# nico-franco-gomez/dsptoolbox

Measured on AMD Instinct MI355X. Metric: Msamples/s + GB/s vs HBM roofline, 64ch Welch H1 nfft=4096 @1/2/4/8 GPU, higher is better.
Workload: dtype f32

## Files before the change

### dsptoolbox_amd/csrc/kernels_welch4096.hpp

```cpp
#pragma once
#include <hip/hip_runtime.h>
#include <stdint.h>

#include <cmath>
#include <utility>
#include <vector>

#include "kernels_finish.hpp"

namespace welch4096 {

#ifndef W4_ABLATE
#define W4_ABLATE 0
#endif

#ifndef W4_AB
#define W4_AB 0
#endif

#ifndef W4_TIMING
#define W4_TIMING 0
#endif
#if W4_TIMING
__device__ unsigned long long w4_timing[16];
#define W4_TS(i)                                                  \
    do {                                                          \
        __builtin_amdgcn_sched_barrier(0);                        \
        unsigned long long t_ = __builtin_amdgcn_s_memtime();     \
        __builtin_amdgcn_sched_barrier(0);                        \
        if ((i) > 0) w4_ph[(i)-1] += t_ - w4_prev;                \
        w4_prev = t_;                                             \
    } while (0)
#else
#define W4_TS(i)
#endif

constexpr int N = 4096, NT = 256, NB = N / 2 + 1;
constexpr int L1S = 272, L2S = 18;
constexpr int BUF_C = 256 * L2S;
constexpr int LDS_BYTES = BUF_C * 8 + 256 * 8;
constexpr int LDS_BYTES_2 = 2 * BUF_C * 8 + 256 * 8;

__device__ __forceinline__ float2 cmul(float2 a, float2 b) {
    return make_float2(fmaf(a.x, b.x, -a.y * b.y), fmaf(a.x, b.y, a.y * b.x));
}

__device__ __forceinline__ void r4(float2& a, float2& b, float2& c, float2& d) {
    float2 s0 = make_float2(a.x + c.x, a.y + c.y), d0 = make_float2(a.x - c.x, a.y - c.y);
    float2 s1 = make_float2(b.x + d.x, b.y + d.y), d1 = make_float2(b.x - d.x, b.y - d.y);
    a = make_float2(s0.x + s1.x, s0.y + s1.y);
    c = make_float2(s0.x - s1.x, s0.y - s1.y);
    b = make_float2(d0.x + d1.y, d0.y - d1.x);
    d = make_float2(d0.x - d1.y, d0.y + d1.x);
}

__device__ __forceinline__ void dft16(float2 (&v)[16]) {
    constexpr float C8 = 0.92387953251128673848f, S8 = 0.38268343236508978178f;
    constexpr float R2 = 0.70710678118654752440f;
#pragma unroll
    for (int n0 = 0; n0 < 4; ++n0) r4(v[n0], v[n0 + 4], v[n0 + 8], v[n0 + 12]);
    auto mulw = [](float2 z, float c, float s) {
        return make_float2(fmaf(z.x, c, z.y * s), fmaf(z.y, c, -z.x * s));
    };
    v[1 + 4] = mulw(v[1 + 4], C8, S8);
    v[1 + 8] = make_float2((v[9].x + v[9].y) * R2, (v[9].y - v[9].x) * R2);
    v[1 + 12] = mulw(v[1 + 12], S8, C8);
    v[2 + 4] = make_float2((v[6].x + v[6].y) * R2, (v[6].y - v[6].x) * R2);
    v[2 + 8] = make_float2(v[10].y, -v[10].x);
    v[2 + 12] = make_float2((v[14].y - v[14].x) * R2, -(v[14].x + v[14].y) * R2);
    v[3 + 4] = mulw(v[3 + 4], S8, C8);
    v[3 + 8] = make_float2((v[11].y - v[11].x) * R2, -(v[11].x + v[11].y) * R2);
    v[3 + 12] = mulw(v[3 + 12], -C8, -S8);
#pragma unroll
    for (int k1 = 0; k1 < 4; ++k1) r4(v[4 * k1], v[4 * k1 + 1], v[4 * k1 + 2], v[4 * k1 + 3]);
}
__device__ __forceinline__ constexpr int pos16(int k) { return 4 * (k & 3) + (k >> 2); }

#define W4_PIN() __builtin_amdgcn_sched_barrier(0)
template <typename PA, typename HA, typename HB>
__device__ __forceinline__ void dft16_h(float2 (&v)[16], PA pre_a, HA after_a, HB after_b) {
    constexpr float C8 = 0.92387953251128673848f, S8 = 0.38268343236508978178f;
    constexpr float R2 = 0.70710678118654752440f;
    auto mulw = [](float2 z, float c, float s) {
        return make_float2(fmaf(z.x, c, z.y * s), fmaf(z.y, c, -z.x * s));
    };
    pre_a(std::integral_constant<int, 0>{});
    r4(v[0], v[4], v[8], v[12]);
    after_a(0);
    pre_a(std::integral_constant<int, 1>{});
    r4(v[1], v[5], v[9], v[13]);
    if (!(W4_AB & 16)) {
    v[5] = mulw(v[5], C8, S8);
    v[9] = make_float2((v[9].x + v[9].y) * R2, (v[9].y - v[9].x) * R2);
    v[13] = mulw(v[13], S8, C8);
    }
    after_a(1);
    pre_a(std::integral_constant<int, 2>{});
    r4(v[2], v[6], v[10], v[14]);
    if (!(W4_AB & 16)) {
    v[6] = make_float2((v[6].x + v[6].y) * R2, (v[6].y - v[6].x) * R2);
    v[10] = make_float2(v[10].y, -v[10].x);
    v[14] = make_float2((v[14].y - v[14].x) * R2, -(v[14].x + v[14].y) * R2);
    }
    after_a(2);
    pre_a(std::integral_constant<int, 3>{});
    r4(v[3], v[7], v[11], v[15]);
    if (!(W4_AB & 16)) {
    v[7] = mulw(v[7], S8, C8);
    v[11] = make_float2((v[11].y - v[11].x) * R2, -(v[11].x + v[11].y) * R2);
    v[15] = mulw(v[15], -C8, -S8);
    }
    after_a(3);
#pragma unroll
    for (int g = 0; g < 4; ++g) {
        r4(v[4 * g], v[4 * g + 1], v[4 * g + 2], v[4 * g + 3]);
        after_b(g);
    }
}
struct NoHookI {
    template <typename T>
    __device__ __forceinline__ void operator()(T) const {}
};


struct Tw {
    float2 w[15];
};

struct NoHook {
    __device__ __forceinline__ void operator()() const {}
};
template <bool TWO_BUF, typename Hook = NoHook, typename Hook2 = NoHook>
__device__ __forceinline__ void fft4096(float2 (&v)[16], const Tw& tw, float2* __restrict__ buf,
                                        const float2* __restrict__ tw2, int tid
#if W4_TIMING
                                        , unsigned long long (&w4_ph)[12], unsigned long long& w4_prev
#endif
                                        , Hook behind_ex1 = Hook(), Hook2 behind_ex2 = Hook2()) {
    float2* __restrict__ bufB = TWO_BUF ? buf + BUF_C : buf;
    dft16(v);
#pragma unroll
    for (int k1 = 1; k1 < 16; ++k1) v[pos16(k1)] = cmul(v[pos16(k1)], tw.w[k1 - 1]);
    W4_TS(2);
    const int k1u = tid >> 4, n3 = tid & 15;
    if (!(W4_ABLATE & 4)) {
        if (!TWO_BUF) __syncthreads();
#pragma unroll
        for (int k1 = 0; k1 < 16; ++k1) buf[k1 * L1S + tid] = v[pos16(k1)];
    }
    float2 w2[15];
#pragma unroll
    for (int k2 = 1; k2 < 16; ++k2) w2[k2 - 1] = tw2[k2 * 16 + n3];
    behind_ex1();
    if (!(W4_ABLATE & 4)) {
        W4_TS(3);
        __syncthreads();
        W4_TS(4);
#pragma unroll
        for (int n2 = 0; n2 < 16; ++n2) v[n2] = buf[k1u * L1S + 16 * n2 + n3];
    }
    W4_TS(5);
    dft16(v);
#pragma unroll
    for (int k2 = 1; k2 < 16; ++k2) v[pos16(k2)] = cmul(v[pos16(k2)], w2[k2 - 1]);
    W4_TS(6);
    if (!(W4_ABLATE & 4)) {
        if (!TWO_BUF) __syncthreads();
#pragma unroll
        for (int k2 = 0; k2 < 16; ++k2) bufB[(16 * k2 + k1u) * L2S + n3] = v[pos16(k2)];
        behind_ex2();
        W4_TS(7);
        __syncthreads();
        W4_TS(8);
        const float4* row = reinterpret_cast<const float4*>(bufB + tid * L2S);
#pragma unroll
        for (int j = 0; j < 8; ++j) {
            float4 r = row[j];
            v[2 * j] = make_float2(r.x, r.y);
            v[2 * j + 1] = make_float2(r.z, r.w);
        }
    }
    W4_TS(9);
    dft16(v);
    W4_TS(10);
}

template <bool TWO_BUF>
__device__ __forceinline__ void fft4096_plain(float2 (&v)[16], const Tw& tw, float2* __restrict__ buf,
                                              const float2* __restrict__ tw2, int tid) {
#if W4_TIMING
    unsigned long long ph[12] = {}, prev = 0;
    fft4096<TWO_BUF>(v, tw, buf, tw2, tid, ph, prev);
#else
    fft4096<TWO_BUF>(v, tw, buf, tw2, tid);
#endif
}

struct Args {
    const float* sig;
    int64_t n_samples, ld;
    int n_ch, hop, n_frames, n_pairs, detrend;
    int n_chunks, ppc;
    const float* window;
    const float2* twt;
    float2* xs;
    float* px;
    float2* pxy;
    float* pyy;
    float* psx;
    int use_plus;
    uint32_t plus[24];
    int n_cx;
    const float* xsig;
};

constexpr int TWT_LEN = 15 * 256 + 256;
__device__ __forceinline__ void init_tables(Tw& tw, float (&win)[16], float2* tw2,
                                            const float* __restrict__ window,
                                            const float2* __restrict__ twt, int tid) {
#pragma unroll
    for (int k1 = 1; k1 < 16; ++k1) tw.w[k1 - 1] = twt[(k1 - 1) * 256 + tid];
#pragma unroll
    for (int n1 = 0; n1 < 16; ++n1) win[n1] = window[tid + 256 * n1];
    tw2[tid] = twt[15 * 256 + tid];
    __syncthreads();
}
inline void host_tables(std::vector<float2>& t) {
    t.resize(TWT_LEN);
    for (int k1 = 1; k1 < 16; ++k1)
        for (int tt = 0; tt < 256; ++tt) {
            double a = -2.0 * M_PI * (double)(tt * k1) / 4096.0;
            t[(k1 - 1) * 256 + tt] = make_float2((float)std::cos(a), (float)std::sin(a));
        }
    for (int k2 = 0; k2 < 16; ++k2)
        for (int n3 = 0; n3 < 16; ++n3) {
            double a = -2.0 * M_PI * (double)(n3 * k2) / 256.0;
            t[15 * 256 + k2 * 16 + n3] = make_float2((float)std::cos(a), (float)std::sin(a));
        }
}

template <bool HALF_HOP>
struct Raw {
    float s[HALF_HOP ? 24 : 32];
};

template <bool HALF_HOP>
__device__ __forceinline__ void load_raw(Raw<HALF_HOP>& r, const float* __restrict__ ch,
                                         int64_t n_samples, int64_t start0, int hop, int tid) {
    const float* __restrict__ src = ch + start0;
    const int64_t remain = n_samples - start0;
    const int span = HALF_HOP ? 3 * 2048 : hop + 4096;
    if (remain >= span) {
        if (HALF_HOP) {
#pragma unroll
            for (int m = 0; m < 24; ++m) r.s[m] = src[tid + 256 * m];
        } else {
#pragma unroll
            for (int n1 = 0; n1 < 16; ++n1) {
                r.s[n1] = src[tid + 256 * n1];
                r.s[16 + n1] = src[hop + tid + 256 * n1];
            }
        }
    } else {
        const int last = (int)(remain > (int64_t)(1 << 30) ? (1 << 30) : remain) - 1;
        constexpr int CNT = HALF_HOP ? 24 : 32;
#pragma unroll
        for (int m = 0; m < CNT; ++m) {
            int i = HALF_HOP ? tid + 256 * m : (m < 16 ? tid + 256 * m : hop + tid + 256 * (m - 16));
            float a = src[min(i, last)];
            r.s[m] = i <= last ? a : 0.f;
        }
    }
}

template <bool HALF_HOP>
__device__ __forceinline__ void window_pair(float2 (&v)[16], const Raw<HALF_HOP>& r, const float (&win)[16]) {
#pragma unroll
    for (int n1 = 0; n1 < 16; ++n1) {
        float b = HALF_HOP ? r.s[n1 + 8] : r.s[16 + n1];
        v[n1] = make_float2(r.s[n1] * win[n1], b * win[n1]);
    }
}

__device__ __forceinline__ bool needs_drop(const Args& p, int pr) {
    return pr == p.n_pairs - 1 && (p.n_frames & 1) && (int64_t)p.n_frames * p.hop < p.n_samples;
}
__device__ __forceinline__ void drop_second(float2 (&v)[16]) {
#pragma unroll
    for (int n1 = 0; n1 < 16; ++n1) v[n1].y = 0.f;
}

template <bool HALF_HOP>
__global__ __launch_bounds__(NT) void k_x(Args p) {
    extern __shared__ __align__(16) float2 lds[];
    float2* buf = lds;
    float2* tw2 = lds + BUF_C;
    const int tid = threadIdx.x, pr = blockIdx.x, cx = blockIdx.y;
    Tw tw;
    float win[16];
    float2 v[16];
    {
        Raw<HALF_HOP> raw;
        load_raw<HALF_HOP>(raw, p.sig + (int64_t)cx * p.ld, p.n_samples, (int64_t)(2 * pr) * p.hop, p.hop, tid);
        init_tables(tw, win, tw2, p.window, p.twt, tid);
        window_pair<HALF_HOP>(v, raw, win);
        if (needs_drop(p, pr)) drop_second(v);
    }
    fft4096_plain<false>(v, tw, buf, tw2, tid);
    if (p.detrend && tid == 0) v[pos16(0)] = make_float2(0.f, 0.f);
    float4* xo = reinterpret_cast<float4*>(p.xs + ((int64_t)cx * p.n_pairs + pr) * N) + tid;
#pragma unroll
    for (int g = 0; g < 8; ++g) {
        float2 z0 = v[pos16(2 * g)], z1 = v[pos16(2 * g + 1)];
        xo[256 * g] = make_float4(z0.x, z0.y, z1.x, z1.y);
    }
    float* pw = reinterpret_cast<float*>(buf);
    __syncthreads();
#pragma unroll
    for (int k3 = 0; k3 < 16; ++k3) {
        float2 z = v[pos16(k3)];
        pw[tid + 256 * k3] = z.x * z.x + z.y * z.y;
    }
    __syncthreads();
    float* po = p.px + ((int64_t)cx * p.n_pairs + pr) * NB;
    for (int k = tid; k < NB; k += NT) po[k] = 0.5f * (pw[k] + pw[(N - k) & (N - 1)]);
}

template <bool HALF_HOP, bool AUTO = false>
__global__ __launch_bounds__(NT, 2) void k_y(Args p) {
    constexpr bool TWO_BUF = true;
    extern __shared__ __align__(16) float2 lds[];
    float2* buf = lds;
    float2* tw2 = lds + (TWO_BUF ? 2 : 1) * BUF_C;
    const int tid = threadIdx.x;
    int q, c;
    {
        const int b = blockIdx.x;
        if ((p.n_chunks & 7) == 0) {
            const int per = p.n_chunks >> 3;
            q = (b & 7) + 8 * ((b >> 3) % per);
            c = (b >> 3) / per;
        } else {
            q = b % p.n_chunks;
            c = b / p.n_chunks;
        }
    }
    Tw tw;
    float win[16];
    init_tables(tw, win, tw2, p.window, p.twt, tid);
    const float* ch = p.sig + (int64_t)c * p.ld;
    const int p0 = (int)((int64_t)q * p.n_pairs / p.n_chunks), p1 = (int)((int64_t)(q + 1) * p.n_pairs / p.n_chunks);
    if (!AUTO && p.n_cx <= 1) {
        double* red = reinterpret_cast<double*>(lds);
        const int bpc = (NB + p.n_ch - 1) / p.n_ch;
        const int b0 = c * bpc, b1 = min(b0 + bpc, NB);
        const int rg = tid >> 5, kl = tid & 31;
        for (int kb = b0; kb < b1; kb += 32) {
            const int k = kb + kl;
            double sum = 0.0;
            if (k < b1)
                for (int pr = p0 + rg; pr < p1; pr += 8) sum += (double)p.px[(int64_t)pr * NB + k];
            red[rg * 32 + kl] = sum;
            __syncthreads();
            if (rg == 0 && k < b1) {
                double t = 0.0;
#pragma unroll
                for (int j = 0; j < 8; ++j) t += red[j * 32 + kl];
                p.psx[(int64_t)q * NB + k] = (float)t;
            }
            __syncthreads();
        }
    }
    float2 T[16];
    float P[16];
#pragma unroll
    for (int j = 0; j < 16; ++j) {
        T[j] = make_float2(0.f, 0.f);
        P[j] = 0.f;
    }
    if constexpr (TWO_BUF) {
        Raw<HALF_HOP> raw;
        if (p0 < p1) load_raw<HALF_HOP>(raw, ch, p.n_samples, (int64_t)(2 * p0) * p.hop, p.hop, tid);
#if W4_TIMING
        unsigned long long w4_ph[12] = {}, w4_prev = 0;
#endif
        for (int pr = p0; pr < p1; ++pr) {
            float2 v[16];
            W4_TS(0);
            window_pair<HALF_HOP>(v, raw, win);
            if (needs_drop(p, pr)) drop_second(v);
            float2 xw[16];
            auto issue_loads = [&]() {
                __builtin_amdgcn_sched_barrier(0);
                if (!(W4_ABLATE & 2) && pr + 1 < p1)
                    load_raw<HALF_HOP>(raw, ch, p.n_samples, (int64_t)(2 * pr + 2) * p.hop, p.hop, tid);
                __builtin_amdgcn_sched_barrier(0);
            };
            auto issue_xs = [&]() {
                if (AUTO) return;
                __builtin_amdgcn_sched_barrier(0);
                if (W4_ABLATE & 1) {
#pragma unroll
                    for (int k3 = 0; k3 < 16; ++k3) xw[k3] = tw.w[k3 % 15];
                } else {
                    const float4* __restrict__ xp =
                        reinterpret_cast<const float4*>(p.xs + ((int64_t)(p.n_cx > 1 ? c : 0) * p.n_pairs + pr) * N) + tid;
#pragma unroll
                    for (int g = 0; g < 8; ++g) {
                        float4 q = xp[256 * g];
                        xw[2 * g] = make_float2(q.x, q.y);
                        xw[2 * g + 1] = make_float2(q.z, q.w);
                    }
                }
                __builtin_amdgcn_sched_barrier(0);
            };
            W4_TS(1);
#if W4_TIMING
            fft4096<TWO_BUF>(v, tw, buf, tw2, tid, w4_ph, w4_prev, issue_loads, issue_xs);
#else
            fft4096<TWO_BUF>(v, tw, buf, tw2, tid, issue_loads, issue_xs);
#endif
#pragma unroll
            for (int k3 = 0; k3 < 16; ++k3) {
                float2 z = v[pos16(k3)];
                if (!AUTO) {
                    float2 w = xw[k3];
                    T[k3].x = fmaf(w.x, z.x, fmaf(w.y, z.y, T[k3].x));
                    T[k3].y = fmaf(w.x, z.y, fmaf(-w.y, z.x, T[k3].y));
                }
                P[k3] = fmaf(z.x, z.x, fmaf(z.y, z.y, P[k3]));
            }
            W4_TS(11);
        }
#if W4_TIMING
        if (blockIdx.x == 0 && tid == 0) {
            for (int i = 0; i < 11; ++i) atomicAdd(&w4_timing[i], w4_ph[i]);
            atomicAdd(&w4_timing[15], (unsigned long long)(p1 - p0));
        }
#endif
    }
    if (p.detrend && tid == 0) P[0] = 0.f;
    __syncthreads();
    const int64_t so = ((int64_t)q * p.n_ch + c) * NB;
    if (!AUTO) {
#pragma unroll
        for (int k3 = 0; k3 < 16; ++k3) buf[tid + 256 * k3] = T[k3];
        __syncthreads();
        for (int k = tid; k < NB; k += NT) {
            float2 a = buf[k], b = buf[(N - k) & (N - 1)];
            p.pxy[so + k] = make_float2(0.5f * (a.x + b.x), 0.5f * (a.y - b.y));
        }
        __syncthreads();
    }
    float* pw = reinterpret_cast<float*>(buf);
#pragma unroll
    for (int k3 = 0; k3 < 16; ++k3) pw[tid + 256 * k3] = P[k3];
    __syncthreads();
    for (int k = tid; k < NB; k += NT) p.pyy[so + k] = 0.5f * (pw[k] + pw[(N - k) & (N - 1)]);
}

inline int chunks_for(int n_pairs, int n_ch, int want = 0) {
    if (want <= 0) {
        want = (512 + n_ch - 1) / n_ch;
        want = (want + 7) & ~7;
        int by_len = (n_pairs + 63) / 64;
        if (want < by_len) want = (by_len + 7) & ~7;
    }
    if (want > n_pairs) want = n_pairs;
    if (want >= 8) want &= ~7;
    if (want < 1) want = 1;
    return want;
}

struct Plan {
    int n_pairs, n_chunks, ppc;
};
inline Plan plan(int n_frames, int n_cy, int want_chunks = 0) {
    Plan pl;
    pl.n_pairs = (n_frames + 1) / 2;
    pl.n_chunks = chunks_for(pl.n_pairs, n_cy, want_chunks);
    pl.ppc = (pl.n_pairs + pl.n_chunks - 1) / pl.n_chunks;
    return pl;
}

}
```

### dsptoolbox_amd/csrc/kernels_welch4096w.hpp

```cpp
#pragma once
#include <utility>

#include "kernels_welch4096.hpp"

namespace welch4096 {

#if W4_TIMING
__device__ unsigned long long w3_timing[16];
__device__ unsigned long long w3_life[4096][8];
struct Stamp {
    unsigned long long ph[12] = {}, prev = 0;
    __device__ __forceinline__ void operator()(int i) {
        __builtin_amdgcn_sched_barrier(0);
        unsigned long long t;
        asm volatile("s_memtime %0\n\ts_waitcnt lgkmcnt(0)" : "=s"(t)::"memory");
        __builtin_amdgcn_sched_barrier(0);
        if (i > 0) ph[i - 1] += t - prev;
        prev = t;
    }
};
#else
struct Stamp {
    __device__ __forceinline__ void operator()(int) {}
};
#endif

constexpr int L3S = 17;
constexpr int LDS3_BYTES = 16 * L1S * 8 + 256 * 8 + N * 4;

__device__ __forceinline__ void wave_sync() {
    __builtin_amdgcn_fence(__ATOMIC_RELEASE, "wavefront");
    __builtin_amdgcn_wave_barrier();
    __builtin_amdgcn_fence(__ATOMIC_ACQUIRE, "wavefront");
}

#ifndef W4_OCC
#define W4_OCC 3
#endif
#ifndef W4_WIN_ROT
#define W4_WIN_ROT 1
#endif
#ifndef W4_TW6
#define W4_TW6 (W4_OCC == 3)
#endif
#ifndef W4_NO_READ2
#define W4_NO_READ2 1
#endif
#ifndef W4_TW2_REG
#define W4_TW2_REG 0
#endif
#ifndef W4_WIN_GLOBAL
#define W4_WIN_GLOBAL 0
#endif
constexpr int LDS3G_BYTES = 16 * L1S * 8 + 256 * 8;

struct Tw6 {
#if W4_TW6
    float2 a[3];
    float2 b[3];
#else
    float2 w[15];
#endif
#if W4_TW2_REG
    float2 c[3];
    float2 d[3];
#endif
};

__device__ __forceinline__ void load_tw6(Tw6& tw, const float2* __restrict__ twt, int tid) {
#if W4_TW6
#pragma unroll
    for (int j = 0; j < 3; ++j) {
        tw.a[j] = twt[j * 256 + tid];
        tw.b[j] = twt[(4 * (j + 1) - 1) * 256 + tid];
    }
#else
#pragma unroll
    for (int k1 = 1; k1 < 16; ++k1) tw.w[k1 - 1] = twt[(k1 - 1) * 256 + tid];
#endif
#if W4_TW2_REG
#pragma unroll
    for (int j = 0; j < 3; ++j) {
        tw.c[j] = twt[15 * 256 + (j + 1) * 16 + (tid & 15)];
        tw.d[j] = twt[15 * 256 + 4 * (j + 1) * 16 + (tid & 15)];
    }
#endif
}

__device__ __forceinline__ void apply_tw6(float2 (&v)[16], const Tw6& tw) {
#if W4_TW6
#pragma unroll
    for (int k1 = 1; k1 < 16; ++k1) {
        const int lo = k1 & 3, hi = k1 >> 2;
        float2 z = v[pos16(k1)];
        if (lo) z = cmul(z, tw.a[lo - 1]);
        if (hi) z = cmul(z, tw.b[hi - 1]);
        v[pos16(k1)] = z;
    }
#else
#pragma unroll
    for (int k1 = 1; k1 < 16; ++k1) v[pos16(k1)] = cmul(v[pos16(k1)], tw.w[k1 - 1]);
#endif
}

__device__ __forceinline__ __amdgpu_buffer_rsrc_t channel_rsrc(const float* ch, int64_t n_samples) {
    return __builtin_amdgcn_make_buffer_rsrc(const_cast<float*>(ch), 0, (int)(uint32_t)(n_samples * 4), 0x00020000);
}
__device__ __forceinline__ float ld_sample(__amdgpu_buffer_rsrc_t r, int byte_off) {
    return __builtin_bit_cast(float, __builtin_amdgcn_raw_buffer_load_b32(r, byte_off, 0, 0));
}

typedef float v2f_t __attribute__((ext_vector_type(2)));
__device__ __forceinline__ uint32_t lds_addr(const void* p) { return (uint32_t)(uintptr_t)p; }
template <int BYTE_OFF>
__device__ __forceinline__ void lds_rd64(float2& d, uint32_t addr) {
    static_assert(BYTE_OFF >= 0 && BYTE_OFF < 65536 && BYTE_OFF % 8 == 0, "ds_read_b64 offset");
    v2f_t r;
    asm volatile("ds_read_b64 %0, %1 offset:%2" : "=v"(r) : "v"(addr), "n"(BYTE_OFF) : "memory");
    d = make_float2(r.x, r.y);
}
template <int N>
__device__ __forceinline__ void lgkm_wait() {
    static_assert(N >= 0 && N <= 15, "lgkmcnt is a 4-bit counter");
    asm volatile("s_waitcnt lgkmcnt(%0)" ::"n"(N) : "memory");
    __builtin_amdgcn_sched_barrier(0);
}
template <typename F, int... I>
__device__ __forceinline__ void static_for_impl(F&& f, std::integer_sequence<int, I...>) {
    (f(std::integral_constant<int, I>{}), ...);
}
template <int N, typename F>
__device__ __forceinline__ void static_for(F&& f) {
    static_for_impl(static_cast<F&&>(f), std::make_integer_sequence<int, N>{});
}

__device__ __forceinline__ int bin_thread(int tid) { return ((tid & 15) << 4) | (tid >> 4); }
__device__ __forceinline__ int fold_pos(int k) { return k + (k >> 4); }

template <typename Hook = NoHook, typename Hook2 = NoHook>
__device__ __forceinline__ void fft4096_w(float2 (&v)[16], const Tw6& tw, float2* __restrict__ buf,
                                          const float2* __restrict__ tw2, int tid,
                                          Hook behind_ex1 = Hook(), Hook2 behind_ex2 = Hook2()) {
    dft16(v);
    apply_tw6(v, tw);
    const int k1u = tid >> 4, n3 = tid & 15;
    __syncthreads();
#pragma unroll
    for (int k1 = 0; k1 < 16; ++k1) buf[k1 * L1S + tid] = v[pos16(k1)];
    float2 w2[15];
#pragma unroll
    for (int k2 = 1; k2 < 16; ++k2) w2[k2 - 1] = tw2[k2 * 16 + n3];
    behind_ex1();
    __syncthreads();
    float2* __restrict__ row = buf + k1u * L1S;
#pragma unroll
    for (int n2 = 0; n2 < 16; ++n2) v[n2] = row[16 * n2 + n3];
    dft16(v);
#pragma unroll
    for (int k2 = 1; k2 < 16; ++k2) v[pos16(k2)] = cmul(v[pos16(k2)], w2[k2 - 1]);
#pragma unroll
    for (int k2 = 0; k2 < 16; ++k2) row[n3 * L3S + k2] = v[pos16(k2)];
    behind_ex2();
    wave_sync();
#pragma unroll
    for (int j = 0; j < 16; ++j) v[j] = row[j * L3S + n3];
    dft16(v);
}

#ifndef W4_PRIO
#define W4_PRIO 1
#endif
#ifndef W4_XS_EARLY
#define W4_XS_EARLY 0
#endif
#ifndef W4_AB
#define W4_AB 0
#endif
#define W4_SYNC()                          \
    do {                                   \
        if (!(W4_AB & 8)) __syncthreads(); \
    } while (0)
__device__ __forceinline__ void set_prio(int level16, int dither) {
#if W4_PRIO
    const int pr = min(3, (level16 + dither) >> 2);
    if (pr == 0)
        __builtin_amdgcn_s_setprio(0);
    else if (pr == 1)
        __builtin_amdgcn_s_setprio(1);
    else if (pr == 2)
        __builtin_amdgcn_s_setprio(2);
    else
        __builtin_amdgcn_s_setprio(3);
#endif
}

template <typename LA, typename LB, typename MID = NoHook>
__device__ __forceinline__ void fft4096_wi(float2 (&v)[16], const Tw6& tw, float2* __restrict__ buf,
                                           const float2* __restrict__ tw2, int tid, LA ld_a, LB ld_b,
                                           Stamp& ts, int level16, MID mid = MID()) {
    const int k1u = tid >> 4, n3 = tid & 15;
    float2* __restrict__ col = buf + tid;
    dft16_h(
        v, NoHookI(),
        [&](int g) {
            W4_PIN();
            ld_a(g);
            W4_PIN();
        },
        [&](int g) {
#pragma unroll
        for (int j = 0; j < 4; ++j) {
            float2 z = v[4 * g + j];
#if W4_TW6
            if (g) z = cmul(z, tw.a[g - 1]);
            if (j && !((W4_AB & 64) && g)) z = cmul(z, tw.b[j - 1]);
#else
            if (g + 4 * j) z = cmul(z, tw.w[g + 4 * j - 1]);
#endif
            W4_PIN();
            if (W4_AB & 4)
                asm volatile("" ::"v"(z.x), "v"(z.y));
            else
                col[(g + 4 * j) * L1S] = z;
            W4_PIN();
        }
    });
    ts(2);
    W4_SYNC();
    mid();
    ts(3);
    float2* __restrict__ row = buf + k1u * L1S;
    const uint32_t a_row = lds_addr(row + n3), a_tw2 = lds_addr(tw2 + n3);
    W4_PIN();
    static_for<16>([&](auto ic) {
        constexpr int i = decltype(ic)::value, n2 = 4 * (i & 3) + (i >> 2);
        if (W4_AB & 4)
            asm volatile("" : "=v"(v[n2].x), "=v"(v[n2].y));
        else
            lds_rd64<16 * n2 * 8>(v[n2], a_row);
    });
    ts(4);
    float2 w2[16];
    dft16_h(
        v,
        [&](auto gc) {
            constexpr int g = decltype(gc)::value;
#if W4_TW2_REG
            lgkm_wait<12 - 4 * g>();
#else
            lgkm_wait<(g == 0 ? 12 : 11)>();
#endif
        },
        [&](int g) {
            W4_PIN();
#if !W4_TW2_REG
            static_for<4>([&](auto jc) {
                constexpr int j = decltype(jc)::value;
                if (g == 0 && j > 0) lds_rd64<(0 + j) * 16 * 8>(w2[0 + j], a_tw2);
                if (g == 1) lds_rd64<(4 + j) * 16 * 8>(w2[4 + j], a_tw2);
                if (g == 2) lds_rd64<(8 + j) * 16 * 8>(w2[8 + j], a_tw2);
                if (g == 3) lds_rd64<(12 + j) * 16 * 8>(w2[12 + j], a_tw2);
            });
#endif
#if W4_XS_EARLY
            ld_b(g);
#endif
            if (g == 3) {
                lgkm_wait<0>();
                ts(5);
            }
            W4_PIN();
        },
        [&](int g) {
#pragma unroll
            for (int j = 0; j < 4; ++j) {
                const int k2 = g + 4 * j;
                float2 z = v[4 * g + j];
#if W4_TW2_REG
                if (g) z = cmul(z, tw.c[g - 1]);
                if (j) z = cmul(z, tw.d[j - 1]);
#else
                if (k2) z = cmul(z, w2[k2]);
#endif
                W4_PIN();
                if (W4_AB & 4)
                    asm volatile("" ::"v"(z.x), "v"(z.y));
                else
                    row[n3 * L3S + k2] = z;
                W4_PIN();
            }
#if !W4_XS_EARLY
            W4_PIN();
            ld_b(g);
            W4_PIN();
#endif
        });
    ts(6);
    wave_sync();
    W4_PIN();
    static_for<16>([&](auto ic) {
        constexpr int i = decltype(ic)::value, j = 4 * (i & 3) + (i >> 2);
        if (W4_AB & 4)
            asm volatile("" : "=v"(v[j].x), "=v"(v[j].y));
        else
            lds_rd64<j * L3S * 8>(v[j], a_row);
    });
    ts(7);
    dft16_h(
        v,
        [&](auto gc) {
            constexpr int g = decltype(gc)::value;
            lgkm_wait<12 - 4 * g>();
            if (g == 3) {
                ts(8);
                W4_SYNC();
                ts(9);
            }
        },
        NoHookI(), NoHookI());
}

__global__ __launch_bounds__(NT) void k_x3(Args p) {
    extern __shared__ __align__(16) float2 lds[];
    float2* buf = lds;
    float2* tw2 = lds + 16 * L1S;
    const int tid = threadIdx.x;
    const int cx = (int)blockIdx.x / p.n_pairs, pr = (int)blockIdx.x - cx * p.n_pairs;
    Tw6 tw;
    float2 v[16];
    {
        Raw<true> raw;
        const __amdgpu_buffer_rsrc_t rs = channel_rsrc(p.sig + (int64_t)cx * p.ld, p.n_samples);
        const int off0 = 4 * (2 * pr * 2048 + tid);
#pragma unroll
        for (int m = 0; m < 24; ++m) raw.s[m] = ld_sample(rs, off0 + 1024 * m);
        float win[16];
        load_tw6(tw, p.twt, tid);
#pragma unroll
        for (int n1 = 0; n1 < 16; ++n1) win[n1] = p.window[tid + 256 * n1];
        tw2[tid] = p.twt[15 * 256 + tid];
        window_pair<true>(v, raw, win);
        if (needs_drop(p, pr)) drop_second(v);
    }
    fft4096_w(v, tw, buf, tw2, tid);
    if (p.detrend && tid == 0) v[pos16(0)] = make_float2(0.f, 0.f);
    float4* xo = reinterpret_cast<float4*>(p.xs + ((int64_t)cx * p.n_pairs + pr) * N) + tid;
#pragma unroll
    for (int g = 0; g < 8; ++g) {
        float2 z0 = v[pos16(2 * g)], z1 = v[pos16(2 * g + 1)];
        xo[256 * g] = make_float4(z0.x, z0.y, z1.x, z1.y);
    }
    float* pw = reinterpret_cast<float*>(buf);
    const int bt = bin_thread(tid);
    __syncthreads();
#pragma unroll
    for (int k3 = 0; k3 < 16; ++k3) {
        float2 z = v[pos16(k3)];
        pw[fold_pos(bt + 256 * k3)] = z.x * z.x + z.y * z.y;
    }
    __syncthreads();
    float* po = p.px + ((int64_t)cx * p.n_pairs + pr) * NB;
    for (int k = tid; k < NB; k += NT) po[k] = 0.5f * (pw[fold_pos(k)] + pw[fold_pos((N - k) & (N - 1))]);
}

__device__ __forceinline__ void chunk_range(const Args& p, int q, int& p0, int& p1) {
    if (p.use_plus) {
        auto below = [&](int qq) {
            int n = 0;
            for (int w = 0; w < (qq >> 5); ++w) n += __popc(p.plus[w]);
            if (qq & 31) n += __popc(p.plus[qq >> 5] & ((1u << (qq & 31)) - 1u));
            return n;
        };
        const int base = p.n_pairs / p.n_chunks;
        p0 = q * base + below(q);
        p1 = p0 + base + (int)((p.plus[q >> 5] >> (q & 31)) & 1u);
    } else {
        p0 = (int)((int64_t)q * p.n_pairs / p.n_chunks);
        p1 = (int)((int64_t)(q + 1) * p.n_pairs / p.n_chunks);
    }
}

__global__ __launch_bounds__(256) void k_px_sum(Args p) {
    const int q = blockIdx.x, cx = blockIdx.y;
    int p0, p1;
    chunk_range(p, q, p0, p1);
    for (int k = threadIdx.x; k < NB; k += 256) {
        double sum = 0.0;
        for (int pr = p0; pr < p1; ++pr) sum += (double)p.px[((int64_t)cx * p.n_pairs + pr) * NB + k];
        p.psx[((int64_t)q * p.n_cx + cx) * NB + k] = (float)sum;
    }
}

template <bool AUTO = false>
__global__ __launch_bounds__(NT, W4_OCC) void k_y3(Args p) {
    extern __shared__ __align__(16) float2 lds[];
    float2* buf = lds;
    float2* tw2 = lds + 16 * L1S;
    float* winl = reinterpret_cast<float*>(lds + 16 * L1S + 256);
    const int tid = threadIdx.x;
    int q, c;
    {
        const int b = blockIdx.x, total = p.n_chunks * p.n_ch;
        const int u = (total & 7) == 0 ? (b & 7) * (total >> 3) + (b >> 3) : b;
        q = u / p.n_ch;
        c = u - q * p.n_ch;
    }
#if W4_TIMING
    const unsigned long long life_t0 = __builtin_amdgcn_s_memtime(), life_r0 = __builtin_amdgcn_s_memrealtime();
#endif
    Tw6 tw;
    load_tw6(tw, p.twt, tid);
    tw2[tid] = p.twt[15 * 256 + tid];
#if W4_WIN_GLOBAL
    const __amdgpu_buffer_rsrc_t wrs = __builtin_amdgcn_make_buffer_rsrc(const_cast<float*>(p.window), 0, N * 4, 0x00020000);
    (void)winl;
#elif W4_OCC == 3
#pragma unroll
    for (int n1 = 0; n1 < 16; ++n1) winl[tid + 256 * n1] = p.window[tid + 256 * n1];
#else
    float winr[16];
#pragma unroll
    for (int n1 = 0; n1 < 16; ++n1) winr[n1] = p.window[tid + 256 * n1];
#endif
    const float* ch = p.sig + (int64_t)c * p.ld;
    int p0, p1;
    chunk_range(p, q, p0, p1);
    const int cx = p.n_cx > 1 ? c : 0;
    if (!AUTO && p.n_cx <= 1) {
        double* red = reinterpret_cast<double*>(lds);
        const int bpc = (NB + p.n_ch - 1) / p.n_ch;
        const int b0 = c * bpc, b1 = min(b0 + bpc, NB);
        const int lw = bpc <= 32 ? 5 : (bpc <= 64 ? 6 : (bpc <= 128 ? 7 : 8)), width = 1 << lw, rows = NT >> lw;
        const int rg = tid >> lw, kl = tid & (width - 1);
        for (int kb = b0; kb < b1; kb += width) {
            const int k = kb + kl;
            double sum = 0.0;
            if (k < b1)
                for (int pr = p0 + rg; pr < p1; pr += rows) sum += (double)p.px[(int64_t)pr * NB + k];
            red[rg * width + kl] = sum;
            __syncthreads();
            if (rg == 0 && k < b1) {
                double t = 0.0;
                for (int j = 0; j < rows; ++j) t += red[j * width + kl];
                p.psx[(int64_t)q * NB + k] = (float)t;
            }
            __syncthreads();
        }
    }
    float2 T[16];
    float P[16];
#pragma unroll
    for (int j = 0; j < 16; ++j) {
        T[j] = make_float2(0.f, 0.f);
        P[j] = 0.f;
    }
    float carry[8], nx[16];
    const __amdgpu_buffer_rsrc_t rs = channel_rsrc(ch, p.n_samples);
    const __amdgpu_buffer_rsrc_t xrs =
        AUTO ? rs
             : __builtin_amdgcn_make_buffer_rsrc(const_cast<float2*>(p.xs + ((int64_t)cx * p.n_pairs + p0) * N), 0,
                                                 (int)(uint32_t)((p1 - p0) * (N * 8)), 0x00020000);
    if (p0 < p1) {
        const int off0 = 4 * (2 * p0 * 2048 + tid);
#pragma unroll
        for (int j = 0; j < 8; ++j) carry[j] = ld_sample(rs, off0 + 1024 * j);
#pragma unroll
        for (int j = 0; j < 16; ++j) nx[j] = ld_sample(rs, off0 + 1024 * (8 + j));
    }
    Stamp ts;
#if W4_TIMING
    const unsigned long long life_r1 = __builtin_amdgcn_s_memrealtime();
#endif
#if W4_WIN_GLOBAL
    float winr[16];
#pragma unroll
    for (int n1 = 0; n1 < 16; ++n1) winr[n1] = ld_sample(wrs, 4 * (tid + 256 * n1));
#elif W4_OCC == 3 && W4_WIN_ROT
    float winr[16];
#pragma unroll
    for (int n1 = 0; n1 < 16; ++n1) winr[n1] = winl[tid + 256 * n1];
#endif
    for (int pr = p0; pr < p1; ++pr) {
        float2 v[16];
        ts(0);
        const int level16 = ((p1 - pr - 1) * 16) / (p1 - p0);
        set_prio(level16, (pr * 5) & 3);
#pragma unroll
        for (int n1 = 0; n1 < 16; ++n1) {
#if W4_OCC == 3 && !W4_WIN_ROT && !W4_WIN_GLOBAL
            const float w = winl[tid + 256 * n1];
#else
            const float w = winr[n1];
#endif
            const float a = n1 < 8 ? carry[n1] : nx[n1 - 8];
            v[n1] = (W4_AB & 32) ? make_float2(a, nx[n1]) : make_float2(a * w, nx[n1] * w);
        }
#pragma unroll
        for (int j = 0; j < 8; ++j) carry[j] = nx[8 + j];
        if (needs_drop(p, pr)) drop_second(v);
        ts(1);
        float2 xw[16];
        const int off1 = 4 * ((2 * pr + 2) * 2048 + tid) + 1024 * 8;
        const int xoff = (pr - p0) * (N * 8) + tid * 16;
        fft4096_wi(
            v, tw, buf, tw2, tid,
            [&](int g) {
#pragma unroll
                for (int j = 0; j < 4; ++j) {
                    if (W4_AB & 2)
                        asm volatile("" : "=v"(nx[4 * g + j]));
                    else
                        nx[4 * g + j] = ld_sample(rs, off1 + 1024 * (4 * g + j));
                }
            },
            [&](int g) {
#if W4_WIN_GLOBAL
#pragma unroll
                for (int j = 0; j < 4; ++j) winr[4 * g + j] = ld_sample(wrs, 4 * (tid + 256 * (4 * g + j)));
#endif
                if (!AUTO) {
#pragma unroll
                    for (int j = 0; j < 2; ++j) {
                        float4 q4;
                        if (W4_AB & 1)
                            asm volatile("" : "=v"(q4.x), "=v"(q4.y), "=v"(q4.z), "=v"(q4.w));
                        else
                            q4 = __builtin_bit_cast(float4, __builtin_amdgcn_raw_buffer_load_b128(xrs, xoff + 4096 * (2 * g + j), 0, 0));
                        xw[2 * (2 * g + j)] = make_float2(q4.x, q4.y);
                        xw[2 * (2 * g + j) + 1] = make_float2(q4.z, q4.w);
                    }
                }
            },
            ts, level16);
        ts(10);
#pragma unroll
        for (int k3 = 0; k3 < 16; ++k3) {
            float2 z = v[pos16(k3)];
            if (!AUTO) {
                float2 w = xw[k3];
                T[k3].x = fmaf(w.x, z.x, fmaf(w.y, z.y, T[k3].x));
                T[k3].y = fmaf(w.x, z.y, fmaf(-w.y, z.x, T[k3].y));
            }
            P[k3] = fmaf(z.x, z.x, fmaf(z.y, z.y, P[k3]));
        }
#if W4_OCC == 3 && W4_WIN_ROT && !W4_WIN_GLOBAL
        __builtin_amdgcn_sched_barrier(0);
#pragma unroll
        for (int n1 = 0; n1 < 16; ++n1)
            if (!(W4_AB & 32)) winr[n1] = winl[tid + 256 * n1];
        __builtin_amdgcn_sched_barrier(0);
#endif
        ts(11);
    }
#if W4_TIMING
    const unsigned long long life_r2 = __builtin_amdgcn_s_memrealtime();
    if (blockIdx.x == 0 && tid == 0) {
        for (int i = 0; i < 11; ++i) atomicAdd(&w3_timing[i], ts.ph[i]);
        atomicAdd(&w3_timing[15], (unsigned long long)(p1 - p0));
    }
#endif
    if (p.detrend && tid == 0) P[0] = 0.f;
    const int bt = bin_thread(tid);
    __syncthreads();
    const int64_t so = ((int64_t)q * p.n_ch + c) * NB;
    if (!AUTO) {
#pragma unroll
        for (int k3 = 0; k3 < 16; ++k3) buf[fold_pos(bt + 256 * k3)] = T[k3];
        __syncthreads();
        for (int k = tid; k < NB; k += NT) {
            float2 a = buf[fold_pos(k)], b = buf[fold_pos((N - k) & (N - 1))];
            p.pxy[so + k] = make_float2(0.5f * (a.x + b.x), 0.5f * (a.y - b.y));
        }
        __syncthreads();
    }
    float* pw = reinterpret_cast<float*>(buf);
#pragma unroll
    for (int k3 = 0; k3 < 16; ++k3) pw[fold_pos(bt + 256 * k3)] = P[k3];
    __syncthreads();
    for (int k = tid; k < NB; k += NT) p.pyy[so + k] = 0.5f * (pw[fold_pos(k)] + pw[fold_pos((N - k) & (N - 1))]);
#if W4_TIMING
    if (tid == 0 && blockIdx.x < 4096) {
        w3_life[blockIdx.x][0] = life_t0;
        w3_life[blockIdx.x][1] = __builtin_amdgcn_s_memtime();
        w3_life[blockIdx.x][2] = life_r0;
        w3_life[blockIdx.x][3] = __builtin_amdgcn_s_memrealtime();
        w3_life[blockIdx.x][4] = life_r1;
        w3_life[blockIdx.x][5] = life_r2;
        w3_life[blockIdx.x][6] = __builtin_amdgcn_s_getreg((4) | (0 << 6) | (31 << 11));
        w3_life[blockIdx.x][7] = __builtin_amdgcn_s_getreg((20) | (0 << 6) | (31 << 11));
    }
#endif
}

inline int chunks_for3(int n_pairs, int n_ch, int want = 0) {
    if (want <= 0) {
        want = (768 + n_ch - 1) / n_ch;
        const int by_len = (n_pairs + 63) / 64;
        if (want < by_len) want = by_len;
        for (int w = want; w < want + 8; ++w)
            if (((int64_t)w * n_ch) % 8 == 0) {
                want = w;
                break;
            }
    }
    if (want > n_pairs) want = n_pairs;
    if (want < 1) want = 1;
    return want;
}
inline Plan plan3(int n_frames, int n_cy, int want_chunks = 0) {
    Plan pl;
    pl.n_pairs = (n_frames + 1) / 2;
    pl.n_chunks = chunks_for3(pl.n_pairs, n_cy, want_chunks);
    pl.ppc = (pl.n_pairs + pl.n_chunks - 1) / pl.n_chunks;
    return pl;
}
inline void place_remainder(Args& a, int n_ch) {
    a.use_plus = 0;
    for (auto& w : a.plus) w = 0;
    const int nc = a.n_chunks, total = nc * n_ch;
    if (nc > 24 * 32 || (total & 7) != 0 || nc <= 0) return;
    const int base = a.n_pairs / nc, rem = a.n_pairs - base * nc;
    a.use_plus = 1;
    if (rem == 0) return;
    const int U = total / 8;
    std::vector<int> ov((size_t)8 * nc, 0);
    for (int u = 0; u < total; ++u) ov[(size_t)(u / U) * nc + u / n_ch] += 1;
    std::vector<int64_t> load(8, 0);
    for (int x = 0; x < 8; ++x)
        for (int q = 0; q < nc; ++q) load[x] += (int64_t)ov[(size_t)x * nc + q] * base;
    std::vector<char> taken(nc, 0);
    for (int r = 0; r < rem; ++r) {
        int best = -1;
        int64_t best_max = 0, best_aff = 0;
        for (int q = 0; q < nc; ++q) {
            if (taken[q]) continue;
            int64_t mx = 0, aff = 0;
            for (int x = 0; x < 8; ++x) {
                const int64_t l = load[x] + ov[(size_t)x * nc + q];
                mx = std::max(mx, l);
                if (ov[(size_t)x * nc + q]) aff = std::max(aff, l);
            }
            if (best < 0 || mx < best_max || (mx == best_max && aff < best_aff)) {
                best = q;
                best_max = mx;
                best_aff = aff;
            }
        }
        taken[best] = 1;
        a.plus[best >> 5] |= 1u << (best & 31);
        for (int x = 0; x < 8; ++x) load[x] += ov[(size_t)x * nc + best];
    }
}

inline bool fits3(int64_t n_samples, int n_frames) {
    return n_samples < ((int64_t)1 << 30) - 8192 && (int64_t)(n_frames + 2) * 2048 < ((int64_t)1 << 30) - 8192;
}

}
```

Baseline: 636,800.

## Replace final LDS transpose stage of 4096-point FFT with DPP row rotation

Adds a new FFT variant that folds a per-thread rotation into the first-stage and second-stage twiddle tables. The last 16-point stage then reads its inputs through DPP row_ror lane rotations instead of a second LDS exchange. Output indexing moves to a reversed position map (posr16), and the twiddle table grows with the rotated factors. The goal is to cut one LDS round trip and barrier per FFT. In exchange it adds extra complex multiplies, DPP moves and a changed result ordering that must match the accumulation step exactly.

```diff
diff --git a/dsptoolbox_amd/csrc/kernels_welch4096.hpp b/dsptoolbox_amd/csrc/kernels_welch4096.hpp
--- a/dsptoolbox_amd/csrc/kernels_welch4096.hpp
+++ b/dsptoolbox_amd/csrc/kernels_welch4096.hpp
@@ -214,7 +214,8 @@
     const float* xsig;
 };
 
-constexpr int TWT_LEN = 15 * 256 + 256;
+constexpr int TWT_R = 16 * 256;
+constexpr int TWT_LEN = TWT_R + 5 * 256;
 __device__ __forceinline__ void init_tables(Tw& tw, float (&win)[16], float2* tw2,
                                             const float* __restrict__ window,
                                             const float2* __restrict__ twt, int tid) {
@@ -236,6 +237,20 @@
         for (int n3 = 0; n3 < 16; ++n3) {
             double a = -2.0 * M_PI * (double)(n3 * k2) / 256.0;
             t[15 * 256 + k2 * 16 + n3] = make_float2((float)std::cos(a), (float)std::sin(a));
+        }
+    for (int tt = 0; tt < 256; ++tt) {
+        const int rot = ((tt >> 4) * (tt & 15)) & 15;
+        for (int k1 = 1; k1 < 4; ++k1) {
+            double a = -2.0 * M_PI * (double)(tt * k1 + 256 * rot) / 4096.0;
+            t[TWT_R + (k1 - 1) * 256 + tt] = make_float2((float)std::cos(a), (float)std::sin(a));
+        }
+        double a = -2.0 * M_PI * (double)rot / 16.0;
+        t[TWT_R + 3 * 256 + tt] = make_float2((float)std::cos(a), (float)std::sin(a));
+    }
+    for (int m = 0; m < 16; ++m)
+        for (int n3 = 0; n3 < 16; ++n3) {
+            double a = -2.0 * M_PI * (double)(n3 * ((m + n3) & 15)) / 256.0;
+            t[TWT_R + 4 * 256 + m * 16 + n3] = make_float2((float)std::cos(a), (float)std::sin(a));
         }
 }
 
diff --git a/dsptoolbox_amd/csrc/kernels_welch4096w.hpp b/dsptoolbox_amd/csrc/kernels_welch4096w.hpp
--- a/dsptoolbox_amd/csrc/kernels_welch4096w.hpp
+++ b/dsptoolbox_amd/csrc/kernels_welch4096w.hpp
@@ -320,13 +320,109 @@
         NoHookI(), NoHookI());
 }
 
+struct Tw6R {
+    float2 a[3];
+    float2 b[3];
+    float2 c;
+};
+constexpr int TW2R = TWT_R + 4 * 256;
+
+__device__ __forceinline__ void load_tw6r(Tw6R& tw, const float2* __restrict__ twt, int tid) {
+#pragma unroll
+    for (int j = 0; j < 3; ++j) {
+        tw.a[j] = twt[TWT_R + j * 256 + tid];
+        tw.b[j] = twt[(4 * (j + 1) - 1) * 256 + tid];
+    }
+    tw.c = twt[TWT_R + 3 * 256 + tid];
+}
+
+__device__ __forceinline__ constexpr int posr16(int k3) { return pos16((16 - k3) & 15); }
+
+template <int R>
+__device__ __forceinline__ float2 row_ror(float2 z) {
+    if constexpr (R == 0) {
+        return z;
+    } else {
+        const int x = __builtin_amdgcn_update_dpp(0, __float_as_int(z.x), 0x120 + R, 0xf, 0xf, true);
+        const int y = __builtin_amdgcn_update_dpp(0, __float_as_int(z.y), 0x120 + R, 0xf, 0xf, true);
+        return make_float2(__int_as_float(x), __int_as_float(y));
+    }
+}
+
+template <typename LA, typename LB>
+__device__ __forceinline__ void fft4096_wr(float2 (&v)[16], const Tw6R& tw, float2* __restrict__ buf,
+                                           const float2* __restrict__ tw2r, int tid, LA ld_a, LB ld_b) {
+    const int k1u = tid >> 4, n3 = tid & 15;
+    float2* __restrict__ col = buf + tid;
+    dft16_h(
+        v, NoHookI(),
+        [&](int g) {
+            W4_PIN();
+            ld_a(g);
+            W4_PIN();
+        },
+        [&](int g) {
+#pragma unroll
+            for (int j = 0; j < 4; ++j) {
+                float2 z = cmul(v[4 * g + j], g ? tw.a[g - 1] : tw.c);
+                if (j) z = cmul(z, tw.b[j - 1]);
+                W4_PIN();
+                col[(g + 4 * j) * L1S] = z;
+                W4_PIN();
+            }
+        });
+    W4_SYNC();
+    const uint32_t a_row = lds_addr(buf + k1u * L1S + n3), a_tw2 = lds_addr(tw2r + n3);
+    W4_PIN();
+    static_for<16>([&](auto ic) {
+        constexpr int i = decltype(ic)::value, n2 = 4 * (i & 3) + (i >> 2);
+        lds_rd64<16 * n2 * 8>(v[n2], a_row);
+    });
+    float2 w2[16];
+    dft16_h(
+        v,
+        [&](auto) {
+            lgkm_wait<12>();
+        },
+        [&](int g) {
+            W4_PIN();
+            static_for<4>([&](auto jc) {
+                constexpr int j = decltype(jc)::value;
+                if (g == 0) lds_rd64<(0 + j) * 16 * 8>(w2[0 + j], a_tw2);
+                if (g == 1) lds_rd64<(4 + j) * 16 * 8>(w2[4 + j], a_tw2);
+                if (g == 2) lds_rd64<(8 + j) * 16 * 8>(w2[8 + j], a_tw2);
+                if (g == 3) lds_rd64<(12 + j) * 16 * 8>(w2[12 + j], a_tw2);
+            });
+            if (g == 3) {
+                lgkm_wait<0>();
+                W4_SYNC();
+            }
+            W4_PIN();
+        },
+        [&](int g) {
+#pragma unroll
+            for (int j = 0; j < 4; ++j) v[4 * g + j] = cmul(v[4 * g + j], w2[g + 4 * j]);
+            W4_PIN();
+            ld_b(g);
+            W4_PIN();
+        });
+    float2 u[16];
+    static_for<16>([&](auto mc) {
+        constexpr int m = decltype(mc)::value;
+        u[m] = row_ror<m>(v[pos16(m)]);
+    });
+#pragma unroll
+    for (int m = 0; m < 16; ++m) v[m] = u[m];
+    dft16(v);
+}
+
 __global__ __launch_bounds__(NT) void k_x3(Args p) {
     extern __shared__ __align__(16) float2 lds[];
     float2* buf = lds;
     float2* tw2 = lds + 16 * L1S;
     const int tid = threadIdx.x;
     const int cx = (int)blockIdx.x / p.n_pairs, pr = (int)blockIdx.x - cx * p.n_pairs;
-    Tw6 tw;
+    Tw6R tw;
     float2 v[16];
     {
         Raw<true> raw;
@@ -335,19 +431,19 @@
 #pragma unroll
         for (int m = 0; m < 24; ++m) raw.s[m] = ld_sample(rs, off0 + 1024 * m);
         float win[16];
-        load_tw6(tw, p.twt, tid);
+        load_tw6r(tw, p.twt, tid);
 #pragma unroll
         for (int n1 = 0; n1 < 16; ++n1) win[n1] = p.window[tid + 256 * n1];
-        tw2[tid] = p.twt[15 * 256 + tid];
+        tw2[tid] = p.twt[TW2R + tid];
         window_pair<true>(v, raw, win);
         if (needs_drop(p, pr)) drop_second(v);
     }
-    fft4096_w(v, tw, buf, tw2, tid);
-    if (p.detrend && tid == 0) v[pos16(0)] = make_float2(0.f, 0.f);
+    fft4096_wr(v, tw, buf, tw2, tid, NoHookI(), NoHookI());
+    if (p.detrend && tid == 0) v[posr16(0)] = make_float2(0.f, 0.f);
     float4* xo = reinterpret_cast<float4*>(p.xs + ((int64_t)cx * p.n_pairs + pr) * N) + tid;
 #pragma unroll
     for (int g = 0; g < 8; ++g) {
-        float2 z0 = v[pos16(2 * g)], z1 = v[pos16(2 * g + 1)];
+        float2 z0 = v[posr16(2 * g)], z1 = v[posr16(2 * g + 1)];
         xo[256 * g] = make_float4(z0.x, z0.y, z1.x, z1.y);
     }
     float* pw = reinterpret_cast<float*>(buf);
@@ -355,7 +451,7 @@
     __syncthreads();
 #pragma unroll
     for (int k3 = 0; k3 < 16; ++k3) {
-        float2 z = v[pos16(k3)];
+        float2 z = v[posr16(k3)];
         pw[fold_pos(bt + 256 * k3)] = z.x * z.x + z.y * z.y;
     }
     __syncthreads();
@@ -408,9 +504,9 @@
 #if W4_TIMING
     const unsigned long long life_t0 = __builtin_amdgcn_s_memtime(), life_r0 = __builtin_amdgcn_s_memrealtime();
 #endif
-    Tw6 tw;
-    load_tw6(tw, p.twt, tid);
-    tw2[tid] = p.twt[15 * 256 + tid];
+    Tw6R tw;
+    load_tw6r(tw, p.twt, tid);
+    tw2[tid] = p.twt[TW2R + tid];
 #if W4_WIN_GLOBAL
     const __amdgpu_buffer_rsrc_t wrs = __builtin_amdgcn_make_buffer_rsrc(const_cast<float*>(p.window), 0, N * 4, 0x00020000);
     (void)winl;
@@ -502,7 +598,7 @@
         float2 xw[16];
         const int off1 = 4 * ((2 * pr + 2) * 2048 + tid) + 1024 * 8;
         const int xoff = (pr - p0) * (N * 8) + tid * 16;
-        fft4096_wi(
+        fft4096_wr(
             v, tw, buf, tw2, tid,
             [&](int g) {
 #pragma unroll
@@ -530,12 +626,11 @@
                         xw[2 * (2 * g + j) + 1] = make_float2(q4.z, q4.w);
                     }
                 }
-            },
-            ts, level16);
+            });
         ts(10);
 #pragma unroll
         for (int k3 = 0; k3 < 16; ++k3) {
-            float2 z = v[pos16(k3)];
+            float2 z = v[posr16(k3)];
             if (!AUTO) {
                 float2 w = xw[k3];
                 T[k3].x = fmaf(w.x, z.x, fmaf(w.y, z.y, T[k3].x));
```

Result: faster. 648,600, median of 6 (+1.9%).
